# iiscleap/ICL-speech-text-LLM

Hardware: AMD Instinct MI355X
Metric: ICL utterances/sec (whole node), SALMONN+Llama2-7B 5-shot VOXCELEB (higher is better)
Workload: dtype bf16

## Files before the change

### icl-speech-text-llm_amd/csrc/gemm.hip

```cpp
#include "gemm_common.h"

using namespace iclg;

namespace {


#define TILE_STAGES_DEEP(BM_, BN_) (((BM_) + (BN_)) <= 128 ? 4 : 3)

template <int WAVES_M, int WAVES_N, int MI, int NI, int NST>
__global__ __launch_bounds__(256) void gemm_bf16_kernel(GemmParams p) {
  constexpr int BM = WAVES_M * MI * 16, BN = WAVES_N * NI * 16;
  constexpr int A_BYTES = BM * 128, W_BYTES = BN * 128, BUF = A_BYTES + W_BYTES;
  constexpr int A_INSTR = BM / 32, W_INSTR = BN / 32;
  constexpr int G_STAGE = A_INSTR + W_INSTR;
  static_assert(WAVES_M * WAVES_N == 4, "4 waves per block");
  extern __shared__ __attribute__((aligned(16))) char smem[];

  const int tid = threadIdx.x, lane = tid & 63;
  const int wave = __builtin_amdgcn_readfirstlane(tid >> 6);
  const int wm = wave / WAVES_N, wn = wave % WAVES_N;

  int tm, tn;
  block_to_tile(p, blockIdx.x, tm, tn);
  const int m0 = tm * BM, n0 = tn * BN;

  const int z = blockIdx.z;
  const __bf16* A = p.A;
  int kt0 = 0, kt1 = p.K >> 6;
  if (p.split_k > 1) {
    const int nk = p.K >> 6;
    kt0 = (int)(((int64_t)z * nk) / p.split_k);
    kt1 = (int)(((int64_t)(z + 1) * nk) / p.split_k);
  } else {
    A += (int64_t)z * p.sA;
  }

  const __bf16* ga[A_INSTR];
  const __bf16* gw[W_INSTR];
#pragma unroll
  for (int j = 0; j < A_INSTR; ++j) {
    const int row = (j * 4 + wave) * 8 + (lane >> 3);
    const int chunk = (lane & 7) ^ ((row >> 1) & 7);
    const int gm = min(m0 + row, p.M - 1);
    ga[j] = A + (int64_t)gm * p.lda + chunk * 8;
  }
#pragma unroll
  for (int j = 0; j < W_INSTR; ++j) {
    const int row = (j * 4 + wave) * 8 + (lane >> 3);
    const int chunk = (lane & 7) ^ ((row >> 1) & 7);
    const int gn = min(n0 + row, p.N - 1);
    gw[j] = p.W + (int64_t)gn * p.ldw + chunk * 8;
  }

  auto stage = [&](int buf_off, int kt) {
    char* base = smem + buf_off;
#pragma unroll
    for (int j = 0; j < A_INSTR; ++j)
      __builtin_amdgcn_global_load_lds((gptr_t)(ga[j] + (int64_t)kt * 64),
                                       (lptr_t)(base + (j * 4 + wave) * 1024), 16, 0, 0);
#pragma unroll
    for (int j = 0; j < W_INSTR; ++j)
      __builtin_amdgcn_global_load_lds((gptr_t)(gw[j] + (int64_t)kt * 64),
                                       (lptr_t)(base + A_BYTES + (j * 4 + wave) * 1024), 16, 0, 0);
  };

  const int fr = lane & 15, fq = lane >> 4;
  int a_off[2], w_off[2];
#pragma unroll
  for (int kk = 0; kk < 2; ++kk) {
    const int sw = ((kk * 4 + fq) ^ (fr >> 1)) * 16;
    a_off[kk] = (wm * MI * 16 + fr) * 128 + sw;
    w_off[kk] = (wn * NI * 16 + fr) * 128 + sw;
  }

  f32x4 acc[MI][NI];
#pragma unroll
  for (int i = 0; i < MI; ++i)
#pragma unroll
    for (int j = 0; j < NI; ++j) acc[i][j] = f32x4{0.f, 0.f, 0.f, 0.f};

  const bool vecp = p.split_k == 1 && vec_path_ok(p);
  const bool interior = vecp && (m0 + BM <= p.M) && (n0 + BN <= p.N);
  const bool fold_bias = vecp && (p.epi & ICL_EPI_BIAS);
// ... 41 lines not shown
          for (int j = 0; j < NI; ++j)
            acc[i][j] = __builtin_amdgcn_mfma_f32_16x16x32_bf16(wf[j], af[i], acc[i][j], 0, 0, 0);
      }
      fill = cur;
      cur = cur == (NST - 1) * BUF ? 0 : cur + BUF;
    }
    asm volatile("s_waitcnt vmcnt(0)" ::: "memory");
  }

  if (interior) {
    const int mb = m0 + wm * MI * 16 + fr, nb = n0 + wn * NI * 16 + fq * 4;
    if (p.epi & ICL_EPI_SWIGLU) {
      if constexpr (NI % 2 == 0) {
#pragma unroll
        for (int i = 0; i < MI; ++i)
#pragma unroll
          for (int j = 0; j < NI; j += 2) {
            f32x4 v;
#pragma unroll
            for (int r = 0; r < 4; ++r) v[r] = silu_f(acc[i][j][r]) * acc[i][j + 1][r];
            store_out4(p, (int64_t)z * p.sC + (int64_t)(mb + i * 16) * p.ldc + ((n0 + wn * NI * 16 + j * 16) >> 1) + fq * 4, v);
          }
      }
      return;
    }
    const bool late_res = p.epi & ICL_EPI_RESIDUAL;
    f32x4 rv[MI][NI];
    if (late_res) {
#pragma unroll
      for (int i = 0; i < MI; ++i)
#pragma unroll
        for (int j = 0; j < NI; ++j)
          rv[i][j] = load_res4(p, (int64_t)z * p.sR + (int64_t)(mb + i * 16) * p.ldr + nb + j * 16);
    }
#pragma unroll
    for (int i = 0; i < MI; ++i)
#pragma unroll
      for (int j = 0; j < NI; ++j) {
        f32x4 v = acc[i][j];
        if (p.epi & ICL_EPI_GELU) {
            v = gelu_erf4(v);
        }
        if (late_res) v = v + rv[i][j];
        store_out4(p, (int64_t)z * p.sC + (int64_t)(mb + i * 16) * p.ldc + nb + j * 16, v);
      }
    return;
  }
  GemmParams q = p;
  if (fold_bias) q.epi &= ~ICL_EPI_BIAS;
#pragma unroll
  for (int i = 0; i < MI; ++i) {
    const int m = m0 + wm * MI * 16 + i * 16 + fr;
#pragma unroll
    for (int j = 0; j < NI; ++j) {
      const int nt = n0 + wn * NI * 16 + j * 16;
      if (p.split_k > 1) {
        epi_store_partial(p, z, m, nt + fq * 4, acc[i][j]);
      } else if (p.epi & ICL_EPI_SWIGLU) {
        if constexpr (NI % 2 == 0) {
          if ((j & 1) == 0) epi_store_swiglu(q, z, m, nt, fq * 4, acc[i][j], acc[i][j + 1]);
        }
      } else {
        epi_store4(q, z, m, nt + fq * 4, acc[i][j]);
      }
    }
  }
}

__device__ __forceinline__ f32x4 sum_slabs4(const float* src, int64_t slab, int split) {
  f32x4 v = {0.f, 0.f, 0.f, 0.f};
  int s = 0;
  for (; s + 4 <= split; s += 4) {
    const f32x4 a = *(const f32x4*)(src + (s + 0) * slab), b = *(const f32x4*)(src + (s + 1) * slab);
    const f32x4 c = *(const f32x4*)(src + (s + 2) * slab), d = *(const f32x4*)(src + (s + 3) * slab);
    v = v + a;
    v = v + b;
    v = v + c;
    v = v + d;
  }
  for (; s < split; ++s) v = v + *(const f32x4*)(src + s * slab);
  return v;
}

__global__ __launch_bounds__(256) void gemm_splitk_reduce_kernel(GemmParams p) {
  const bool swiglu = p.epi & ICL_EPI_SWIGLU;
  const int Nout = swiglu ? p.N / 2 : p.N;
  const int64_t total = (int64_t)p.M * Nout;
  const int64_t slab = (int64_t)p.M * p.N;
  const bool vec = (p.N & 31) == 0 && (p.ldc & 3) == 0 && (!(p.epi & ICL_EPI_RESIDUAL) || ((p.ldr & 3) == 0 && p.res_dtype == ICL_F32)) &&
                   (((uintptr_t)p.ws | (uintptr_t)p.C) & 15) == 0 && (!(p.epi & ICL_EPI_BIAS) || ((uintptr_t)p.bias & 15) == 0) &&
                   (!(p.epi & ICL_EPI_RESIDUAL) || ((uintptr_t)p.R & 15) == 0);
  if (vec) {
    const int nq = Nout >> 2;
    const int64_t total4 = (int64_t)p.M * nq;
    for (int64_t idx = (int64_t)blockIdx.x * blockDim.x + threadIdx.x; idx < total4; idx += (int64_t)gridDim.x * blockDim.x) {
      const int m = (int)(idx / nq), c = (int)(idx % nq) * 4;
      f32x4 v;
      if (swiglu) {
        const int ng = (c >> 4) * 32 + (c & 15), nu = ng + 16;
        f32x4 g = sum_slabs4(p.ws + (int64_t)m * p.N + ng, slab, p.split_k);
        f32x4 u = sum_slabs4(p.ws + (int64_t)m * p.N + nu, slab, p.split_k);
        if (p.epi & ICL_EPI_BIAS) {
          g = g + *(const f32x4*)(p.bias + ng);
          u = u + *(const f32x4*)(p.bias + nu);
        }
#pragma unroll
        for (int r = 0; r < 4; ++r) v[r] = silu_f(g[r]) * u[r];
      } else {
        v = sum_slabs4(p.ws + (int64_t)m * p.N + c, slab, p.split_k);
        if (p.epi & ICL_EPI_BIAS) v = v + *(const f32x4*)(p.bias + c);
        if (p.epi & ICL_EPI_GELU) v = gelu_erf4(v);
        if (p.epi & ICL_EPI_RESIDUAL) v = v + *(const f32x4*)((const float*)p.R + (int64_t)m * p.ldr + c);
      }
      const int64_t coff = (int64_t)m * p.ldc + c;
      if (p.out_dtype == ICL_BF16) *(u32x2*)((unsigned short*)p.C + coff) = u32x2{pack_bf16x2(v[0], v[1]), pack_bf16x2(v[2], v[3])};
      else *(f32x4*)((float*)p.C + coff) = v;
    }
    return;
  }
  for (int64_t idx = (int64_t)blockIdx.x * blockDim.x + threadIdx.x; idx < total;
       idx += (int64_t)gridDim.x * blockDim.x) {
    const int m = (int)(idx / Nout), c = (int)(idx % Nout);
    float v;
    if (swiglu) {
      const int ng = (c >> 4) * 32 + (c & 15), nu = ng + 16;
      float g = 0.f, u = 0.f;
      for (int s = 0; s < p.split_k; ++s) {
        g += p.ws[s * slab + (int64_t)m * p.N + ng];
        u += p.ws[s * slab + (int64_t)m * p.N + nu];
      }
      if (p.epi & ICL_EPI_BIAS) {
        g += p.bias[ng];
        u += p.bias[nu];
      }
      v = silu_f(g) * u;
    } else {
      v = 0.f;
      for (int s = 0; s < p.split_k; ++s) v += p.ws[s * slab + (int64_t)m * p.N + c];
      if (p.epi & ICL_EPI_BIAS) v += p.bias[c];
      if (p.epi & ICL_EPI_GELU) v = gelu_erf(v);
      if (p.epi & ICL_EPI_RESIDUAL) {
        const int64_t roff = (int64_t)m * p.ldr + c;
        v += (p.res_dtype == ICL_F32) ? ((const float*)p.R)[roff]
                                      : bf16_bits_to_f32(((const unsigned short*)p.R)[roff]);
      }
    }
    const int64_t coff = (int64_t)m * p.ldc + c;
    if (p.out_dtype == ICL_BF16)
      ((unsigned short*)p.C)[coff] = f32_to_bf16_bits(v);
    else
      ((float*)p.C)[coff] = v;
  }
}



template <int VPT>
__global__ __launch_bounds__(256) void splitk_reduce_rmsnorm_kernel(GemmParams p, const float* gamma, float eps,
                                                                    unsigned short* xn, int64_t ldx) {
  __shared__ float wsum[4];
  const int m = blockIdx.x, tid = threadIdx.x, nvec = p.N >> 2;
  const int64_t slab = (int64_t)p.M * p.N;
  const bool store_c = p.split_k > 1 || p.ws != (const float*)p.C;
  f32x4 v[VPT];
#pragma unroll
  for (int i = 0; i < VPT; ++i) {
    const int c = tid + i * 256;
    v[i] = f32x4{0.f, 0.f, 0.f, 0.f};
    if (c < nvec) v[i] = sum_slabs4(p.ws + (int64_t)m * p.N + c * 4, slab, p.split_k);
  }
  float ss = 0.f;
#pragma unroll
  for (int i = 0; i < VPT; ++i) {
    const int c = tid + i * 256;
    if (c < nvec) {
      if (p.epi & ICL_EPI_RESIDUAL) v[i] = v[i] + *(const f32x4*)((const float*)p.R + (int64_t)m * p.ldr + c * 4);
      if (store_c) *(f32x4*)((float*)p.C + (int64_t)m * p.ldc + c * 4) = v[i];
      ss += v[i][0] * v[i][0] + v[i][1] * v[i][1] + v[i][2] * v[i][2] + v[i][3] * v[i][3];
    }
  }
  ss = wave_reduce_sum(ss);
  if ((tid & 63) == 0) wsum[tid >> 6] = ss;
  __syncthreads();
  const float rstd = rsqrtf((((wsum[0] + wsum[1]) + wsum[2]) + wsum[3]) / (float)p.N + eps);
#pragma unroll
  for (int i = 0; i < VPT; ++i) {
    const int c = tid + i * 256;
    if (c < nvec) {
      const f32x4 g = *(const f32x4*)(gamma + c * 4);
      const f32x4 o = v[i] * rstd * g;
      *(u32x2*)(xn + (int64_t)m * ldx + c * 4) = u32x2{pack_bf16x2(o[0], o[1]), pack_bf16x2(o[2], o[3])};
    }
  }
}


template <int WAVES_M, int WAVES_N, int MI, int NI, int NST>
int launch_tile_n(GemmParams& p, dim3 grid, hipStream_t stream) {
  constexpr int BM = WAVES_M * MI * 16, BN = WAVES_N * NI * 16;
  constexpr int SMEM = (BM + BN) * 128 * NST;
  if (const int rc = allow_dynamic_lds<gemm_bf16_kernel<WAVES_M, WAVES_N, MI, NI, NST>>(SMEM)) return rc;
  hipLaunchKernelGGL((gemm_bf16_kernel<WAVES_M, WAVES_N, MI, NI, NST>), grid, dim3(256), SMEM, stream, p);
  ICL_CHECK_LAUNCH("icl_gemm_bf16");
  return ICL_OK;
}

template <int WAVES_M, int WAVES_N, int MI, int NI>
int launch_tile(GemmParams& p, int batch, hipStream_t stream) {
  constexpr int BM = WAVES_M * MI * 16, BN = WAVES_N * NI * 16;
  constexpr int DEEP = TILE_STAGES_DEEP(BM, BN);
  p.tiles_m = (p.M + BM - 1) / BM;
  p.tiles_n = (p.N + BN - 1) / BN;
  dim3 grid(p.tiles_m * p.tiles_n, 1, p.split_k > 1 ? p.split_k : batch);
  static int n_cu = 0;
  if (n_cu <= 0) {
    n_cu = icl_device_cu_count();
    if (n_cu <= 0) n_cu = 256;
  }
  const int64_t blocks = (int64_t)grid.x * grid.z;
  const int per_cu = (160 * 1024) / ((BM + BN) * 128 * DEEP);
  if (blocks <= (int64_t)n_cu * per_cu) return launch_tile_n<WAVES_M, WAVES_N, MI, NI, DEEP>(p, grid, stream);
  return launch_tile_n<WAVES_M, WAVES_N, MI, NI, 2>(p, grid, stream);
}

struct NormFuse {
  const float* gamma;
  float eps;
  unsigned short* xn;
  int64_t ldx;
};

void launch_reduce_rmsnorm(const GemmParams& p, const NormFuse& nf, hipStream_t stream) {
  auto kern = p.N <= 4096 ? splitk_reduce_rmsnorm_kernel<4> : splitk_reduce_rmsnorm_kernel<8>;
  hipLaunchKernelGGL(kern, dim3(p.M), dim3(256), 0, stream, p, nf.gamma, nf.eps, nf.xn, nf.ldx);
}

}


extern "C" int icl_gemm_select_tile(int32_t M, int32_t N, int32_t K, int32_t batch, int32_t split_k) {
  const int64_t t128 = (int64_t)((M + 127) / 128) * ((N + 127) / 128) * batch;
  if (split_k > 1 || M <= 64 || t128 < 256) return 2;
  if (N <= 64) return 2;
  if (N <= 128) return 1;
  static int ncu = 0;
  if (ncu <= 0) {
    ncu = icl_device_cu_count();
    if (ncu <= 0) ncu = 256;
  }
  const int64_t t256 = (int64_t)((M + 255) / 256) * ((N + 255) / 256) * batch;
  const int64_t rounds = (t256 + ncu - 1) / ncu;
  const double eff = (double)t256 / (double)(rounds * ncu);
  if (K >= 768 && eff >= 0.6) return 3;
  return 1;
}

static int gemm_impl(const icl_gemm_args* a, void* stream_, const RopeFuse* rope, const NormFuse* norm = nullptr,
                     const float* wscale = nullptr) {
  hipStream_t stream = (hipStream_t)stream_;
  ICL_CHECK_ARG(a != nullptr, "icl_gemm_bf16: args is NULL");
  ICL_CHECK_ARG(a->A && a->W && a->C, "icl_gemm_bf16: A/W/C must be non-NULL");
  ICL_CHECK_ARG(a->M > 0 && a->N > 0 && a->K > 0, "icl_gemm_bf16: M,N,K must be > 0 (got %d,%d,%d)",
                a->M, a->N, a->K);
  ICL_CHECK_ARG(a->K % 64 == 0, "icl_gemm_bf16: K=%d must be a multiple of 64", a->K);
  ICL_CHECK_ARG(a->lda % 8 == 0 && a->ldw % 8 == 0,
                "icl_gemm_bf16: lda=%lld / ldw=%lld must be multiples of 8", (long long)a->lda,
                (long long)a->ldw);
  ICL_CHECK_ARG(((uintptr_t)a->A & 15) == 0 && ((uintptr_t)a->W & 15) == 0,
                "icl_gemm_bf16: A and W must be 16-byte aligned");
  ICL_CHECK_ARG(a->ldw >= a->K, "icl_gemm_bf16: ldw=%lld < K=%d", (long long)a->ldw, a->K);
  ICL_CHECK_ARG(a->batch >= 1 && a->batch <= 65535, "icl_gemm_bf16: batch=%d out of range", a->batch);
  ICL_CHECK_ARG(a->split_k >= 1 && a->split_k <= 64, "icl_gemm_bf16: split_k=%d out of range", a->split_k);
  ICL_CHECK_ARG(a->out_dtype == ICL_BF16 || a->out_dtype == ICL_F32, "icl_gemm_bf16: bad out_dtype %d",
                a->out_dtype);
  ICL_CHECK_ARG(a->res_dtype == ICL_BF16 || a->res_dtype == ICL_F32, "icl_gemm_bf16: bad res_dtype %d",
                a->res_dtype);
  ICL_CHECK_ARG((a->epilogue & ~15) == 0, "icl_gemm_bf16: unknown epilogue bits 0x%x", a->epilogue);
  const bool swiglu = a->epilogue & ICL_EPI_SWIGLU;
  if (swiglu) {
    ICL_CHECK_ARG(a->N % 32 == 0, "icl_gemm_bf16: SWIGLU needs N %% 32 == 0 (N=%d)", a->N);
    ICL_CHECK_ARG((a->epilogue & (ICL_EPI_GELU | ICL_EPI_RESIDUAL)) == 0,
                  "icl_gemm_bf16: SWIGLU cannot be combined with GELU/RESIDUAL");
    ICL_CHECK_ARG(a->ldc % 4 == 0, "icl_gemm_bf16: SWIGLU needs ldc %% 4 == 0");
  }
  if (a->epilogue & ICL_EPI_BIAS) ICL_CHECK_ARG(a->bias, "icl_gemm_bf16: EPI_BIAS without bias");
  if (a->epilogue & ICL_EPI_RESIDUAL) ICL_CHECK_ARG(a->R, "icl_gemm_bf16: EPI_RESIDUAL without R");
  const int nout = swiglu ? a->N / 2 : a->N;
  ICL_CHECK_ARG(a->ldc >= nout, "icl_gemm_bf16: ldc=%lld < %d output columns", (long long)a->ldc, nout);
  if (a->split_k > 1) {
    ICL_CHECK_ARG(a->batch == 1, "icl_gemm_bf16: split_k > 1 requires batch == 1");
    ICL_CHECK_ARG(a->workspace, "icl_gemm_bf16: split_k > 1 requires a workspace");
    ICL_CHECK_ARG(a->split_k <= a->K / 64, "icl_gemm_bf16: split_k=%d > K/64=%d", a->split_k, a->K / 64);
  }
  const int cal = a->out_dtype == ICL_BF16 ? 8 : 16;
  ICL_CHECK_ARG(((uintptr_t)a->C % cal) == 0, "icl_gemm_bf16: C must be %d-byte aligned", cal);
  if (a->R) {
    const int ral = a->res_dtype == ICL_BF16 ? 8 : 16;
    ICL_CHECK_ARG(((uintptr_t)a->R % ral) == 0, "icl_gemm_bf16: R must be %d-byte aligned", ral);
  }

  GemmParams p;
  p.A = (const __bf16*)a->A;
  p.W = (const __bf16*)a->W;
  p.C = a->C;
  p.bias = a->bias;
  p.R = a->R;
  p.ws = a->workspace;
  p.lda = a->lda; p.ldw = a->ldw; p.ldc = a->ldc; p.ldr = a->ldr;
  p.sA = a->strideA; p.sC = a->strideC; p.sR = a->strideR;
  p.M = a->M; p.N = a->N; p.K = a->K;
  p.epi = a->epilogue; p.out_dtype = a->out_dtype; p.res_dtype = a->res_dtype;
  p.split_k = a->split_k;
  p.tiles_m = p.tiles_n = 0;
  p.group_m = p.xcd_sync = 0;

  if (!rope && (wscale || a->tile == 4 || a->tile == 6)) {
    if (!(a->M <= 64 && a->batch == 1)) {
      if (wscale) icl_set_error("icl_gemm_fp8w: needs M <= 64 and batch == 1 (M=%d batch=%d)", a->M, a->batch);
      else icl_set_error("icl_gemm_bf16: the skinny kernel needs M <= 64 and batch == 1");
      return ICL_EINVAL;
    }
    p.split_k = 1;
    return launch_skinny(p, wscale ? SKINNY_W_FP8 : a->tile == 6 ? SKINNY_W_PACKED : SKINNY_W_ROW, wscale, stream);
  }
  int tile = a->tile;
  if (tile == 0) tile = icl_gemm_select_tile(a->M, a->N, a->K, a->batch, a->split_k);
  if (tile == 3 && a->K < 128) tile = 1;
  if (rope) {
    ICL_CHECK_ARG(tile == 3, "icl_gemm_rope_kv_bf16: only the 256x256 tile fuses RoPE (this problem resolves to tile %d; "
                             "use icl_gemm_bf16 + icl_rope_kv_bf16)", tile);
    ICL_CHECK_ARG(a->split_k == 1, "icl_gemm_rope_kv_bf16: split_k must be 1");
    return launch_tile256(p, 1, stream, rope);
  }
  int rc;
  if (tile == 1)
    rc = launch_tile<2, 2, 4, 4>(p, a->batch, stream);
  else if (tile == 2)
    rc = launch_tile<2, 2, 2, 2>(p, a->batch, stream);
  else if (tile == 3) {
    ICL_CHECK_ARG(a->split_k == 1 || (a->split_k <= a->K / 128 && a->N % 4 == 0),
                  "icl_gemm_bf16: split_k=%d on the 256x256 tile needs K / split_k >= 128 and N %% 4 == 0 (K=%d N=%d)", a->split_k, a->K, a->N);
    rc = launch_tile256(p, a->batch, stream);
  } else if (tile == 5) {
    ICL_CHECK_ARG(a->M <= 256 && a->batch == 1, "icl_gemm_bf16: the decode tile needs M <= 256 and batch == 1");
    rc = launch_decode_tile(p, stream);
  } else {
    icl_set_error("icl_gemm_bf16: unsupported tile id %d", tile);
    return ICL_EINVAL;
  }
  if (rc != ICL_OK) return rc;
  if (a->split_k > 1 && norm) {
    launch_reduce_rmsnorm(p, *norm, stream);
    ICL_CHECK_LAUNCH("icl_gemm_rmsnorm_bf16(split-K reduce + RMSNorm)");
  } else if (a->split_k > 1) {
    const int64_t total = (int64_t)a->M * nout;
    int blocks = (int)((total + 255) / 256);
    if (blocks > 2048) blocks = 2048;
    hipLaunchKernelGGL(gemm_splitk_reduce_kernel, dim3(blocks), dim3(256), 0, stream, p);
    ICL_CHECK_LAUNCH("icl_gemm_bf16(split-K reduce)");
  }
  return ICL_OK;
}

extern "C" int icl_rmsnorm(const void* x, int64_t ldx, const float* gamma, void* y, int64_t ldy, int32_t M, int32_t N, float eps,
                           int32_t in_dtype, int32_t out_dtype, void* stream);

static int gemm_rmsnorm_impl(const icl_gemm_args* a, const float* wscale, const float* gamma, float eps, void* xn, int64_t ld_xn,
                             void* stream) {
  ICL_CHECK_ARG(a != nullptr && gamma && xn, "icl_gemm_rmsnorm_bf16: NULL pointer");
  ICL_CHECK_ARG(a->batch == 1 && a->out_dtype == ICL_F32 && (a->epilogue & ~ICL_EPI_RESIDUAL) == 0 &&
                    (!(a->epilogue & ICL_EPI_RESIDUAL) || a->res_dtype == ICL_F32),
                "icl_gemm_rmsnorm_bf16: batch 1, f32 output, residual-only epilogue with an f32 residual");
  ICL_CHECK_ARG(a->N % 4 == 0 && a->N <= 8192 && a->ldc % 4 == 0 && a->ldr % 4 == 0 && ld_xn % 4 == 0 && ld_xn >= a->N,
                "icl_gemm_rmsnorm_bf16: N=%d must be a multiple of 4 and <= 8192, leading dimensions multiples of 4", a->N);
  ICL_CHECK_ARG(((uintptr_t)gamma & 15) == 0 && ((uintptr_t)xn & 7) == 0 && ((uintptr_t)a->C & 15) == 0 &&
                    (!a->R || ((uintptr_t)a->R & 15) == 0), "icl_gemm_rmsnorm_bf16: misaligned pointer");
  if (a->split_k > 1 && a->tile != 4 && a->tile != 6 && !wscale) {
    const NormFuse nf{gamma, eps, (unsigned short*)xn, ld_xn};
    return gemm_impl(a, stream, nullptr, &nf);
  }
  const int rc = gemm_impl(a, stream, nullptr, nullptr, wscale);
  if (rc != ICL_OK) return rc;
#ifndef ICL_SMALL_M_BLOCKNORM
#define ICL_SMALL_M_BLOCKNORM 1
#endif
  if (ICL_SMALL_M_BLOCKNORM && a->M <= 64 && a->ldc == a->N) {
    GemmParams q{};
    q.ws = (float*)a->C; q.C = a->C; q.R = nullptr; q.ldc = a->ldc; q.ldr = 0; q.M = a->M; q.N = a->N; q.split_k = 1; q.epi = 0;
    launch_reduce_rmsnorm(q, NormFuse{gamma, eps, (unsigned short*)xn, ld_xn}, (hipStream_t)stream);
    ICL_CHECK_LAUNCH("icl_gemm_rmsnorm_bf16(row-per-block RMSNorm)");
    return ICL_OK;
  }
  return icl_rmsnorm(a->C, a->ldc, gamma, xn, ld_xn, a->M, a->N, eps, ICL_F32, ICL_BF16, stream);
}

extern "C" int icl_gemm_rmsnorm_bf16(const icl_gemm_args* a, const float* gamma, float eps, void* xn, int64_t ld_xn, void* stream) {
  return gemm_rmsnorm_impl(a, nullptr, gamma, eps, xn, ld_xn, stream);
}

extern "C" int icl_gemm_bf16(const icl_gemm_args* a, void* stream) { return gemm_impl(a, stream, nullptr); }

extern "C" int icl_gemm_fp8w(const icl_gemm_args* a, const float* w_scale, void* stream) {
  ICL_CHECK_ARG(w_scale, "icl_gemm_fp8w: w_scale is NULL");
  return gemm_impl(a, stream, nullptr, nullptr, w_scale);
}

extern "C" int icl_gemm_rmsnorm_fp8w(const icl_gemm_args* a, const float* w_scale, const float* gamma, float eps, void* xn,
                                     int64_t ld_xn, void* stream) {
  ICL_CHECK_ARG(w_scale, "icl_gemm_rmsnorm_fp8w: w_scale is NULL");
  return gemm_rmsnorm_impl(a, w_scale, gamma, eps, xn, ld_xn, stream);
}

extern "C" int icl_gemm_rope_kv_bf16(const icl_gemm_args* a, int64_t k_off, int64_t v_off, const float* cosT,
                                     const float* sinT, const int32_t* pos, const int32_t* seq_ids, void* kcache,
                                     void* vcache, int32_t n_heads, int32_t head_dim, int32_t max_len, int32_t kv_rows_to_c,
                                     void* stream) {
  ICL_CHECK_ARG(a != nullptr && cosT && sinT && pos, "icl_gemm_rope_kv_bf16: NULL pointer");
  ICL_CHECK_ARG(head_dim == 128, "icl_gemm_rope_kv_bf16: head_dim=%d (the fused epilogue is built for 128)", head_dim);
  const int64_t hd = (int64_t)n_heads * 128;
  ICL_CHECK_ARG(n_heads > 0 && hd % 256 == 0 && (k_off == 0 || k_off == hd) && (v_off == k_off || v_off == k_off + hd) &&
                    (a->N == v_off || a->N == v_off + hd) && a->N > 0,
                "icl_gemm_rope_kv_bf16: need q|k|v blocks of n_heads*128 columns each (or empty), a multiple of 256 (N=%d k_off=%lld v_off=%lld)",
                a->N, (long long)k_off, (long long)v_off);
  ICL_CHECK_ARG(a->batch == 1 && a->out_dtype == ICL_BF16 && (a->epilogue & ~ICL_EPI_BIAS) == 0,
                "icl_gemm_rope_kv_bf16: batch 1, bf16 output, bias-only epilogue");
  ICL_CHECK_ARG(a->C && ((uintptr_t)a->C & 15) == 0 && a->ldc % 8 == 0, "icl_gemm_rope_kv_bf16: C must be 16-byte aligned, ldc %% 8 == 0");
  ICL_CHECK_ARG(!a->bias || ((uintptr_t)a->bias & 15) == 0, "icl_gemm_rope_kv_bf16: bias must be 16-byte aligned");
  ICL_CHECK_ARG(((uintptr_t)cosT & 15) == 0 && ((uintptr_t)sinT & 15) == 0, "icl_gemm_rope_kv_bf16: cos/sin misaligned");
  ICL_CHECK_ARG((kcache == nullptr) == (vcache == nullptr), "icl_gemm_rope_kv_bf16: kcache and vcache must both be set or both NULL");
  if (kcache) {
    ICL_CHECK_ARG(seq_ids && max_len > 0, "icl_gemm_rope_kv_bf16: cache append needs seq_ids and max_len");
    ICL_CHECK_ARG(((uintptr_t)kcache & 15) == 0 && ((uintptr_t)vcache & 15) == 0, "icl_gemm_rope_kv_bf16: cache misaligned");
  }
  ICL_CHECK_ARG(kv_rows_to_c || kcache, "icl_gemm_rope_kv_bf16: kv_rows_to_c = 0 needs a cache to hold k / v");
  RopeFuse rf;
  rf.kv_rows_to_c = kv_rows_to_c;
  rf.cosT = cosT; rf.sinT = sinT; rf.pos = pos; rf.seq_ids = seq_ids;
  rf.kc = (unsigned short*)kcache; rf.vc = (unsigned short*)vcache;
  rf.k_off = (int)k_off; rf.v_off = (int)v_off; rf.H = n_heads; rf.max_len = max_len;
  return gemm_impl(a, stream, &rf);
}
// ... 1 lines not shown
```

### icl-speech-text-llm_amd/csrc/gemm256.hip

```cpp
#include "gemm_common.h"
#include <cstdlib>

using namespace iclg;

#ifndef ICL_EPI_NT
#define ICL_EPI_NT 3
#endif

namespace {

constexpr int T256_REGION = 128 * 128;
constexpr int T256_BUF = 4 * T256_REGION;
constexpr int T256_SMEM = 256 * (256 * 2 + 16);

__device__ __forceinline__ void st16(unsigned short* dst, u32x4 v) {
  if (ICL_EPI_NT & 4) __builtin_nontemporal_store(v, (u32x4*)dst);
  else *(u32x4*)dst = v;
}

__device__ __forceinline__ void rope_rows(const GemmParams& p, const RopeFuse& rf, const char* smem, int pitch, int m0,
                                          int n0, int tid) {
  const int sect = n0 >= rf.v_off ? 2 : (n0 >= rf.k_off ? 1 : 0);
  const int head0 = (n0 - (sect == 2 ? rf.v_off : sect == 1 ? rf.k_off : 0)) >> 7;
  unsigned short* C = (unsigned short*)p.C;
  constexpr int U = 4;
  if (sect == 2) {
    for (int base = tid; base < 256 * 32; base += U * 512) {
      int64_t crow[U];
      if (rf.vc) {
#pragma unroll
        for (int u = 0; u < U; ++u) {
          const int m = min(m0 + ((base + u * 512) >> 5), p.M - 1);
          crow[u] = (int64_t)rf.seq_ids[m] * rf.H * rf.max_len + rf.pos[m];
        }
      }
#pragma unroll
      for (int u = 0; u < U; ++u) {
        const int c = base + u * 512, row = c >> 5, cc = c & 31, m = m0 + row;
        if (m >= p.M) continue;
        const u32x4 v = *(const u32x4*)(smem + row * pitch + cc * 16);
        if (rf.kv_rows_to_c) st16(C + (int64_t)m * p.ldc + n0 + cc * 8, v);
        if (rf.vc) st16(rf.vc + (crow[u] + (int64_t)(head0 + (cc >> 4)) * rf.max_len) * 128 + (cc & 15) * 8, v);
      }
    }
    return;
  }
  const bool to_cache = sect == 1 && rf.kc;
  for (int base = tid; base < 256 * 16; base += U * 512) {
    int ps[U], sq[U];
    u32x4 lo[U], hi[U];
    f32x4 c0[U], c1[U], s0[U], s1[U];
#pragma unroll
    for (int u = 0; u < U; ++u) {
      const int m = min(m0 + ((base + u * 512) >> 4), p.M - 1);
      ps[u] = rf.pos[m];
      sq[u] = to_cache ? rf.seq_ids[m] : 0;
    }
#pragma unroll
    for (int u = 0; u < U; ++u) {
      const int it = base + u * 512, row = it >> 4, hh = (it >> 3) & 1, j = it & 7;
      const char* src = smem + row * pitch + hh * 256 + j * 16;
      lo[u] = *(const u32x4*)src;
      hi[u] = *(const u32x4*)(src + 128);
      const float* cp = rf.cosT + (int64_t)ps[u] * 64 + j * 8;
      const float* sp = rf.sinT + (int64_t)ps[u] * 64 + j * 8;
      c0[u] = *(const f32x4*)cp;
      c1[u] = *(const f32x4*)(cp + 4);
      s0[u] = *(const f32x4*)sp;
      s1[u] = *(const f32x4*)(sp + 4);
    }
#pragma unroll
    for (int u = 0; u < U; ++u) {
      const int it = base + u * 512, row = it >> 4, hh = (it >> 3) & 1, j = it & 7, m = m0 + row;
      if (m >= p.M) continue;
      u32x4 olo, ohi;
      rope_rot8(lo[u], hi[u], c0[u], c1[u], s0[u], s1[u], olo, ohi);
      if (sect == 0 || rf.kv_rows_to_c) {
        unsigned short* dst = C + (int64_t)m * p.ldc + n0 + hh * 128 + j * 8;
        st16(dst, olo);
        st16(dst + 64, ohi);
      }
      if (to_cache) {
        unsigned short* cd = rf.kc + (((int64_t)sq[u] * rf.H + head0 + hh) * rf.max_len + ps[u]) * 128 + j * 8;
        st16(cd, olo);
        st16(cd + 64, ohi);
      }
    }
  }
}

constexpr int T256_OUT_F32 = 16;
template <bool ROPE, int EPI>
__global__ __launch_bounds__(512, 2) void gemm256_bf16_kernel(GemmParams p_in, RopeFuse rf) {
  GemmParams p = p_in;
  p.epi = (p_in.epi & ICL_EPI_BIAS) | (EPI & (ICL_EPI_GELU | ICL_EPI_RESIDUAL | ICL_EPI_SWIGLU));
  p.out_dtype = (EPI & T256_OUT_F32) ? ICL_F32 : ICL_BF16;
  extern __shared__ __attribute__((aligned(16))) char smem[];
  const int tid = threadIdx.x, lane = tid & 63;
  const int wave = __builtin_amdgcn_readfirstlane(tid >> 6);
  const int wr = wave >> 2, wc = wave & 3;
  int tm, tn;
  block_to_tile(p, blockIdx.x, tm, tn);
  const int m0 = tm * 256, n0 = tn * 256;
  int z = blockIdx.z;
  int nk = p.K >> 6, kt0 = 0;
  const bool slab_out = p.split_k > 1;
  if (p.split_k > 1) {
    kt0 = (int)(((int64_t)z * nk) / p.split_k);
    nk = (int)(((int64_t)(z + 1) * nk) / p.split_k) - kt0;
    p.C = p.ws + (int64_t)z * p.M * p.N;
    p.ldc = p.N;
    p.sC = 0;
    p.epi = 0;
    z = 0;
  }
  const __bf16* A = p.A + (int64_t)z * p.sA + (int64_t)kt0 * 64;
  const __bf16* Wk = p.W + (int64_t)kt0 * 64;

  const __bf16* gsrc[2][2][2];
#pragma unroll
  for (int h = 0; h < 2; ++h)
#pragma unroll
    for (int r = 0; r < 2; ++r) {
      const int row = (r * 8 + wave) * 8 + (lane >> 3);
      const int chunk = (lane & 7) ^ ((row >> 1) & 7);
      gsrc[0][h][r] = A + (int64_t)min(m0 + h * 128 + row, p.M - 1) * p.lda + chunk * 8;
      gsrc[1][h][r] = Wk + (int64_t)min(n0 + h * 128 + row, p.N - 1) * p.ldw + chunk * 8;
    }
  auto stage = [&](int bo, int which, int h, int kt) {
    const int64_t koff = (int64_t)min(kt, nk - 1) * 64;
    char* base = smem + bo + (which * 2 + h) * T256_REGION + wave * 1024;
    __builtin_amdgcn_global_load_lds((gptr_t)(gsrc[which][h][0] + koff), (lptr_t)(base), 16, 0, 0);
    __builtin_amdgcn_global_load_lds((gptr_t)(gsrc[which][h][1] + koff), (lptr_t)(base + 8 * 1024), 16, 0, 0);
  };

  const int fr = lane & 15, fq = lane >> 4;
  const int a_base = (wr * 64 + fr) * 128, b_base = (wc * 32 + fr) * 128;
  const int sw0 = ((0 + fq) ^ (fr >> 1)) * 16, sw1 = ((4 + fq) ^ (fr >> 1)) * 16;

  f32x4 acc[2][2][4][2];
#pragma unroll
  for (int a = 0; a < 2; ++a)
#pragma unroll
    for (int b = 0; b < 2; ++b)
#pragma unroll
      for (int i = 0; i < 4; ++i)
#pragma unroll
        for (int j = 0; j < 2; ++j) acc[a][b][i][j] = f32x4{0.f, 0.f, 0.f, 0.f};
  bf16x8 af[4][2], b0f[2][2], b1f[2][2];
  const bool vecp = vec_path_ok(p);
  const bool interior = vecp && (m0 + 256 <= p.M) && (n0 + 256 <= p.N);
  const bool fold_bias = vecp && (p.epi & ICL_EPI_BIAS);
  constexpr bool fold_res = false;

  auto read_a = [&](int bo, int h) {
    const char* r = smem + bo + h * T256_REGION + a_base;
#pragma unroll
    for (int i = 0; i < 4; ++i) {
      af[i][0] = *(const bf16x8*)(r + i * 2048 + sw0);
      af[i][1] = *(const bf16x8*)(r + i * 2048 + sw1);
    }
  };
  auto read_b = [&](int bo, int h, bf16x8 (&bf)[2][2]) {
    const char* r = smem + bo + (2 + h) * T256_REGION + b_base;
#pragma unroll
    for (int j = 0; j < 2; ++j) {
      bf[j][0] = *(const bf16x8*)(r + j * 2048 + sw0);
      bf[j][1] = *(const bf16x8*)(r + j * 2048 + sw1);
    }
  };
  auto mma = [&](f32x4 (&c)[4][2], bf16x8 (&bf)[2][2]) {
    __builtin_amdgcn_s_setprio(1);
#pragma unroll
    for (int kk = 0; kk < 2; ++kk)
// ... 21 lines not shown
  auto tile = [&](int bo, int t, auto mode) {
    constexpr int MODE = decltype(mode)::value;
    const int bx = bo ^ T256_BUF;
    read_a(bo, 0);
    read_b(bo, 0, b0f);
    if constexpr (MODE != 2) stage(bx, 1, 1, t + 1);
    phase_sync(std::integral_constant<int, MODE == 2 ? 2 : 8>{});
    mma(acc[0][0], b0f);
    read_b(bo, 1, b1f);
    if constexpr (MODE != 2) stage(bx, 0, 1, t + 1);
    phase_sync(std::integral_constant<int, MODE == 2 ? 0 : 8>{});
    mma(acc[0][1], b1f);
    read_a(bo, 1);
    if constexpr (MODE == 0) stage(bo, 0, 0, t + 2);
    phase_sync(std::integral_constant<int, MODE == 0 ? 8 : (MODE == 1 ? 6 : 0)>{});
    mma(acc[1][1], b1f);
    if constexpr (MODE == 0) stage(bo, 1, 0, t + 2);
    phase_sync(std::integral_constant<int, MODE == 0 ? 8 : (MODE == 1 ? 4 : 0)>{});
    mma(acc[1][0], b0f);
  };
  using M0_ = std::integral_constant<int, 0>;
  using M1_ = std::integral_constant<int, 1>;
  using M2_ = std::integral_constant<int, 2>;

  f32x4 bias_f[2][2];
  if (fold_res) {
#pragma unroll
    for (int qa = 0; qa < 2; ++qa)
#pragma unroll
      for (int qb = 0; qb < 2; ++qb)
#pragma unroll
        for (int i = 0; i < 4; ++i)
#pragma unroll
          for (int j = 0; j < 2; ++j) {
            const int m = m0 + qa * 128 + wr * 64 + i * 16 + fr, n = n0 + qb * 128 + wc * 32 + j * 16 + fq * 4;
            if (interior || (m < p.M && n < p.N))
              acc[qa][qb][i][j] = *(const f32x4*)((const float*)p.R + (int64_t)z * p.sR + (int64_t)m * p.ldr + n);
          }
  }
  if (fold_bias) {
#pragma unroll
    for (int qb = 0; qb < 2; ++qb)
#pragma unroll
      for (int j = 0; j < 2; ++j) {
        const int n = n0 + qb * 128 + wc * 32 + j * 16 + fq * 4;
        bias_f[qb][j] = (interior || n < p.N) ? *(const f32x4*)(p.bias + n) : f32x4{0.f, 0.f, 0.f, 0.f};
      }
  }
  __builtin_amdgcn_sched_barrier(0);
  stage(0, 0, 0, 0);
  stage(0, 1, 0, 0);
  stage(0, 1, 1, 0);
  stage(0, 0, 1, 0);
  stage(T256_BUF, 0, 0, 1);
  stage(T256_BUF, 1, 0, 1);
  __builtin_amdgcn_sched_barrier(0);
  if (fold_bias) {
#pragma unroll
    for (int qa = 0; qa < 2; ++qa)
#pragma unroll
      for (int qb = 0; qb < 2; ++qb)
#pragma unroll
        for (int i = 0; i < 4; ++i)
#pragma unroll
          for (int j = 0; j < 2; ++j) acc[qa][qb][i][j] = acc[qa][qb][i][j] + bias_f[qb][j];
  }
  phase_sync(std::integral_constant<int, 8>{});
  if (wr == 1) __builtin_amdgcn_s_barrier();
  const int n_steady = nk - 2;
  int t = 0;
  for (; t + 1 < n_steady; t += 2) {
    tile(0, t, M0_{});
    tile(T256_BUF, t + 1, M0_{});
  }
  if (t < n_steady) {
    tile(0, t, M0_{});
    ++t;
  }
  const int bo = (t & 1) ? T256_BUF : 0;
  tile(bo, t, M1_{});
  tile(bo ^ T256_BUF, t + 1, M2_{});
  if (wr == 0) __builtin_amdgcn_s_barrier();

  const int es_out = p.out_dtype == ICL_BF16 ? 2 : 4;
  const bool rows16 = (((uintptr_t)p.C | (uintptr_t)(p.ldc * es_out) | (uintptr_t)(p.sC * es_out)) & 15) == 0;
  const bool has_res = p.epi & ICL_EPI_RESIDUAL;
  const bool res_rows = has_res && p.res_dtype == ICL_F32 && p.out_dtype == ICL_F32 && !(p.epi & ICL_EPI_SWIGLU) &&
                        (((uintptr_t)p.R | (uintptr_t)(p.ldr * 4) | (uintptr_t)(p.sR * 4)) & 15) == 0;
  if (ROPE || (interior && rows16 && (!has_res || res_rows))) {
    const bool swiglu = p.epi & ICL_EPI_SWIGLU;
    const bool obf = p.out_dtype == ICL_BF16;
    const int out_cols = swiglu ? 128 : 256;
    const int es = obf ? 2 : 4;
    const int pitch = out_cols * es + 16;
    const int chunks_per_row = out_cols * es / 16;
    const int64_t c_col0 = swiglu ? (n0 >> 1) : n0;
    const bool one_round = ROPE || obf;
    f32x4 rrA[16], rrB[16];
    auto load_res_rows = [&](int qa_, f32x4 (&rr)[16]) {
      const char* rbase = (const char*)p.R + ((int64_t)z * p.sR + (int64_t)(m0 + qa_ * 128) * p.ldr + n0) * 4;
#pragma unroll
      for (int it = 0; it < 16; ++it) {
        const int c = tid + it * 512, row = c >> 6, cc = c & 63;
        rr[it] = ICL_EPI_NT & 1 ? __builtin_nontemporal_load((const f32x4*)(rbase + (int64_t)row * p.ldr * 4 + cc * 16))
                                : *(const f32x4*)(rbase + (int64_t)row * p.ldr * 4 + cc * 16);
      }
    };
    if (has_res) load_res_rows(0, rrA);
#pragma unroll
    for (int qa = 0; qa < 2; ++qa) {
      if (qa == 0 || !one_round) __syncthreads();
      const int row_off = one_round ? qa * 128 : 0;
#pragma unroll
      for (int qb = 0; qb < 2; ++qb)
#pragma unroll
        for (int i = 0; i < 4; ++i) {
          const int row = row_off + wr * 64 + i * 16 + fr;
          if (swiglu) {
            f32x4 v;
#pragma unroll
            for (int r = 0; r < 4; ++r) v[r] = silu_f(acc[qa][qb][i][0][r]) * acc[qa][qb][i][1][r];
            const int col = qb * 64 + wc * 16 + fq * 4;
            char* dst = smem + row * pitch + col * es;
            if (obf) *(u32x2*)dst = u32x2{pack_bf16x2(v[0], v[1]), pack_bf16x2(v[2], v[3])};
            else *(f32x4*)dst = v;
          } else {
#pragma unroll
            for (int j = 0; j < 2; ++j) {
              f32x4 v = acc[qa][qb][i][j];
              if (p.epi & ICL_EPI_GELU) {
            v = gelu_erf4(v);
              }
              const int col = qb * 128 + wc * 32 + j * 16 + fq * 4;
              char* dst = smem + row * pitch + col * es;
              if (obf) *(u32x2*)dst = u32x2{pack_bf16x2(v[0], v[1]), pack_bf16x2(v[2], v[3])};
              else *(f32x4*)dst = v;
            }
          }
        }
      if (one_round && qa == 0) continue;
      __syncthreads();
      if constexpr (ROPE) {
        rope_rows(p, rf, smem, pitch, m0, n0, tid);
        continue;
      }
      char* cbase = (char*)p.C + ((int64_t)z * p.sC + (int64_t)(m0 + (one_round ? 0 : qa * 128)) * p.ldc + c_col0) * es;
      const int n_chunks = (one_round ? 256 : 128) * chunks_per_row;
      if (has_res) {
        if (qa == 0) load_res_rows(1, rrB);
        f32x4 (&rr)[16] = qa == 0 ? rrA : rrB;
#pragma unroll
        for (int it = 0; it < 16; ++it) {
          const int c = tid + it * 512, row = c >> 6, cc = c & 63;
          const f32x4 v = *(const f32x4*)(smem + row * pitch + cc * 16) + rr[it];
          if (ICL_EPI_NT & 1) __builtin_nontemporal_store(v, (f32x4*)(cbase + (int64_t)row * p.ldc * 4 + cc * 16));
          else *(f32x4*)(cbase + (int64_t)row * p.ldc * 4 + cc * 16) = v;
        }
      } else {
        const int n_iter = n_chunks >> 9;
        u32x4 v[16];
#pragma unroll
        for (int it = 0; it < 16; ++it)
          if (it < n_iter) {
            const int c = tid + it * 512, row = c / chunks_per_row, cc = c - row * chunks_per_row;
            v[it] = *(const u32x4*)(smem + row * pitch + cc * 16);
          }
// ... 17 lines not shown
        for (int i = 0; i < 4; ++i)
#pragma unroll
          for (int qb = 0; qb < 2; ++qb) {
            f32x4 v;
#pragma unroll
            for (int r = 0; r < 4; ++r) v[r] = silu_f(acc[qa][qb][i][0][r]) * acc[qa][qb][i][1][r];
            store_out4(p, (int64_t)z * p.sC + (int64_t)(mb + i * 16) * p.ldc + ((n0 + qb * 128 + wc * 32) >> 1) + fq * 4, v);
          }
        continue;
      }
      f32x4 rv[2][4][2];
      if (late_res) {
#pragma unroll
        for (int qb = 0; qb < 2; ++qb)
#pragma unroll
          for (int i = 0; i < 4; ++i)
#pragma unroll
            for (int j = 0; j < 2; ++j)
              rv[qb][i][j] = load_res4(p, (int64_t)z * p.sR + (int64_t)(mb + i * 16) * p.ldr + n0 + qb * 128 + wc * 32 + j * 16 + fq * 4);
      }
#pragma unroll
      for (int qb = 0; qb < 2; ++qb)
#pragma unroll
        for (int i = 0; i < 4; ++i)
#pragma unroll
          for (int j = 0; j < 2; ++j) {
            f32x4 v = acc[qa][qb][i][j];
            if (p.epi & ICL_EPI_GELU) {
            v = gelu_erf4(v);
            }
            if (late_res) v = v + rv[qb][i][j];
            store_out4(p, (int64_t)z * p.sC + (int64_t)(mb + i * 16) * p.ldc + n0 + qb * 128 + wc * 32 + j * 16 + fq * 4, v);
          }
    }
    return;
  }

  GemmParams q = p;
  if (fold_bias) q.epi &= ~ICL_EPI_BIAS;
  if (fold_res) q.epi &= ~ICL_EPI_RESIDUAL;
#pragma unroll
  for (int qa = 0; qa < 2; ++qa)
#pragma unroll
    for (int i = 0; i < 4; ++i) {
      const int m = m0 + qa * 128 + wr * 64 + i * 16 + fr;
#pragma unroll
      for (int qb = 0; qb < 2; ++qb) {
        const int nt = n0 + qb * 128 + wc * 32;
        if (p.epi & ICL_EPI_SWIGLU) {
          epi_store_swiglu(q, z, m, nt, fq * 4, acc[qa][qb][i][0], acc[qa][qb][i][1]);
        } else {
          epi_store4(q, z, m, nt + fq * 4, acc[qa][qb][i][0]);
          epi_store4(q, z, m, nt + 16 + fq * 4, acc[qa][qb][i][1]);
        }
      }
    }
}

template <bool ROPE, int EPI>
int launch256(const GemmParams& p, const dim3& grid, hipStream_t stream, const RopeFuse& rf) {
  auto kern = gemm256_bf16_kernel<ROPE, EPI>;
  if (const int rc = allow_dynamic_lds<gemm256_bf16_kernel<ROPE, EPI>>(T256_SMEM)) return rc;
  hipLaunchKernelGGL(kern, grid, dim3(512), T256_SMEM, stream, p, rf);
  ICL_CHECK_LAUNCH("icl_gemm_bf16(256)");
  return ICL_OK;
}

}

int iclg::launch_tile256(GemmParams& p, int batch, hipStream_t stream, const RopeFuse* rope) {
  p.tiles_m = (p.M + 255) / 256;
  p.tiles_n = (p.N + 255) / 256;
  {
    static const int env_gm = [] { const char* e = getenv("ICL_GEMM_GROUP_M"); return e ? atoi(e) : 0; }();
    static const int env_xs = [] { const char* e = getenv("ICL_GEMM_XCD_SYNC"); return e ? atoi(e) : 1; }();
    const int64_t panel = (int64_t)256 * p.K * 2;
    p.group_m = env_gm > 0 ? env_gm : (int)std::min<int64_t>(6, std::max<int64_t>(1, 8400000 / panel));
    p.xcd_sync = env_xs;
  }
  const dim3 grid(p.tiles_m * p.tiles_n, 1, p.split_k > 1 ? p.split_k : batch);
  if (rope) return launch256<true, 0>(p, grid, stream, *rope);
  const RopeFuse none{};
  constexpr int G = ICL_EPI_GELU, R = ICL_EPI_RESIDUAL, S = ICL_EPI_SWIGLU, F = T256_OUT_F32;
  if (p.split_k > 1) return launch256<false, F>(p, grid, stream, none);
  switch ((p.epi & (G | R | S)) | (p.out_dtype == ICL_F32 ? F : 0)) {
    case 0:         return launch256<false, 0>(p, grid, stream, none);
    case G:         return launch256<false, G>(p, grid, stream, none);
    case R:         return launch256<false, R>(p, grid, stream, none);
    case G | R:     return launch256<false, G | R>(p, grid, stream, none);
    case S:         return launch256<false, S>(p, grid, stream, none);
    case F:         return launch256<false, F>(p, grid, stream, none);
    case F | G:     return launch256<false, F | G>(p, grid, stream, none);
    case F | R:     return launch256<false, F | R>(p, grid, stream, none);
    case F | G | R: return launch256<false, F | G | R>(p, grid, stream, none);
    case F | S:     return launch256<false, F | S>(p, grid, stream, none);
  }
  icl_set_error("icl_gemm_bf16(256): unsupported epilogue combination 0x%x", p.epi);
  return ICL_EINVAL;
}
```

### icl-speech-text-llm_amd/csrc/gemm_common.h

```cpp
#pragma once
#include "common.h"
#include <algorithm>
#include <type_traits>

namespace iclg {


struct GemmParams {
  const __bf16* A;
  const __bf16* W;
  void* C;
  const float* bias;
  const void* R;
  float* ws;
  int64_t lda, ldw, ldc, ldr, sA, sC, sR;
  int M, N, K, epi, out_dtype, res_dtype, split_k, tiles_m, tiles_n;
  int group_m;
  int xcd_sync;
};

constexpr int GROUP_M = 8;

typedef const __attribute__((address_space(1))) void* gptr_t;
typedef __attribute__((address_space(3))) void* lptr_t;


__device__ __forceinline__ void epi_store4(const GemmParams& p, int z, int m, int n, f32x4 acc) {
  if (m >= p.M || n >= p.N) return;
  const bool has_bias = p.epi & ICL_EPI_BIAS, has_gelu = p.epi & ICL_EPI_GELU, has_res = p.epi & ICL_EPI_RESIDUAL;
  char* Cb = (char*)p.C;
  const int64_t cz = (int64_t)z * p.sC, rz = (int64_t)z * p.sR;
  const bool vec_ok = ((p.ldc & 3) == 0) && (!has_res || (p.ldr & 3) == 0);
  float v[4] = {acc[0], acc[1], acc[2], acc[3]};
  const bool full = (n + 3 < p.N);
  if (has_bias) {
#pragma unroll
    for (int r = 0; r < 4; ++r)
      if (full || n + r < p.N) v[r] += p.bias[n + r];
  }
  if (has_gelu) {
    const f32x4 g = gelu_erf4(f32x4{v[0], v[1], v[2], v[3]});
#pragma unroll
    for (int r = 0; r < 4; ++r) v[r] = g[r];
  }
  const int64_t coff = cz + (int64_t)m * p.ldc + n;
  if (full && vec_ok) {
    if (has_res) {
      const int64_t roff = rz + (int64_t)m * p.ldr + n;
      if (p.res_dtype == ICL_F32) {
        f32x4 rv = *(const f32x4*)((const char*)p.R + roff * 4);
#pragma unroll
        for (int r = 0; r < 4; ++r) v[r] += rv[r];
      } else {
        const unsigned short* rp = (const unsigned short*)p.R + roff;
#pragma unroll
        for (int r = 0; r < 4; ++r) v[r] += bf16_bits_to_f32(rp[r]);
      }
    }
    if (p.out_dtype == ICL_BF16) {
      u32x2 pk = {pack_bf16x2(v[0], v[1]), pack_bf16x2(v[2], v[3])};
      *(u32x2*)(Cb + coff * 2) = pk;
    } else {
      *(f32x4*)(Cb + coff * 4) = f32x4{v[0], v[1], v[2], v[3]};
    }
  } else {
#pragma unroll
    for (int r = 0; r < 4; ++r) {
      if (n + r >= p.N) continue;
      float x = v[r];
      if (has_res) {
        const int64_t roff = rz + (int64_t)m * p.ldr + n + r;
        x += (p.res_dtype == ICL_F32) ? ((const float*)p.R)[roff]
                                      : bf16_bits_to_f32(((const unsigned short*)p.R)[roff]);
      }
      if (p.out_dtype == ICL_BF16)
        ((unsigned short*)Cb)[coff + r] = f32_to_bf16_bits(x);
      else
        ((float*)Cb)[coff + r] = x;
    }
  }
}
__device__ __forceinline__ void epi_store_swiglu(const GemmParams& p, int z, int m, int nt, int fq4, f32x4 g4, f32x4 u4) {
  if (m >= p.M || nt >= p.N) return;
  float v[4];
#pragma unroll
  for (int r = 0; r < 4; ++r) {
    float g = g4[r], u = u4[r];
    if (p.epi & ICL_EPI_BIAS) {
      g += p.bias[nt + fq4 + r];
      u += p.bias[nt + 16 + fq4 + r];
    }
    v[r] = silu_f(g) * u;
  }
  const int64_t off = (int64_t)z * p.sC + (int64_t)m * p.ldc + (nt >> 1) + fq4;
  if (p.out_dtype == ICL_BF16) {
    u32x2 pk = {pack_bf16x2(v[0], v[1]), pack_bf16x2(v[2], v[3])};
    *(u32x2*)((char*)p.C + off * 2) = pk;
  } else {
    *(f32x4*)((char*)p.C + off * 4) = f32x4{v[0], v[1], v[2], v[3]};
  }
}
__device__ __forceinline__ void epi_store_partial(const GemmParams& p, int z, int m, int n, f32x4 acc) {
  if (m >= p.M || n >= p.N) return;
  float* dst = p.ws + (int64_t)z * p.M * p.N + (int64_t)m * p.N + n;
// ... 90 lines not shown
```

Baseline: 144.6.

## Store split-K partials in column-blocked slab layout and batch RMSNorm rows per block

The 256x256 split-K GEMM now writes its fp32 partial tiles into a column-blocked (16-column panel) workspace layout through a dedicated epilogue, instead of row-major through the generic F32 epilogue. The split-K reduce and reduce+RMSNorm kernels read that layout, and the reduce kernel walks indices in 4-row by 16-quad blocks. The RMSNorm reduce handles two rows per block. The goal is contiguous, coalesced 64-byte segments on both the partial store and the reduce read. It is on by default, with an environment variable to turn it off, and adds more kernel template instances and indexing arithmetic.

```diff
diff --git a/icl-speech-text-llm_amd/csrc/gemm.hip b/icl-speech-text-llm_amd/csrc/gemm.hip
--- a/icl-speech-text-llm_amd/csrc/gemm.hip
+++ b/icl-speech-text-llm_amd/csrc/gemm.hip
@@ -1,4 +1,5 @@
 #include "gemm_common.h"
+#include <cstdlib>
 
 using namespace iclg;
 
@@ -206,6 +207,7 @@
   return v;
 }
 
+template <bool TILED>
 __global__ __launch_bounds__(256) void gemm_splitk_reduce_kernel(GemmParams p) {
   const bool swiglu = p.epi & ICL_EPI_SWIGLU;
   const int Nout = swiglu ? p.N / 2 : p.N;
@@ -216,14 +218,24 @@
                    (!(p.epi & ICL_EPI_RESIDUAL) || ((uintptr_t)p.R & 15) == 0);
   if (vec) {
     const int nq = Nout >> 2;
-    const int64_t total4 = (int64_t)p.M * nq;
+    const int nqb = (nq + 15) >> 4, nrb = (p.M + 3) >> 2;
+    const int64_t total4 = TILED ? (int64_t)nrb * nqb * 64 : (int64_t)p.M * nq;
     for (int64_t idx = (int64_t)blockIdx.x * blockDim.x + threadIdx.x; idx < total4; idx += (int64_t)gridDim.x * blockDim.x) {
-      const int m = (int)(idx / nq), c = (int)(idx % nq) * 4;
+      int m, c;
+      if constexpr (TILED) {
+        const int blk = (int)(idx >> 6), in = (int)idx & 63;
+        m = (blk % nrb) * 4 + (in >> 4);
+        c = ((blk / nrb) * 16 + (in & 15)) * 4;
+        if (m >= p.M || c >= Nout) continue;
+      } else {
+        m = (int)(idx / nq);
+        c = (int)(idx % nq) * 4;
+      }
       f32x4 v;
       if (swiglu) {
         const int ng = (c >> 4) * 32 + (c & 15), nu = ng + 16;
-        f32x4 g = sum_slabs4(p.ws + (int64_t)m * p.N + ng, slab, p.split_k);
-        f32x4 u = sum_slabs4(p.ws + (int64_t)m * p.N + nu, slab, p.split_k);
+        f32x4 g = sum_slabs4(p.ws + slab_index<TILED>(m, ng, p.M, p.N), slab, p.split_k);
+        f32x4 u = sum_slabs4(p.ws + slab_index<TILED>(m, nu, p.M, p.N), slab, p.split_k);
         if (p.epi & ICL_EPI_BIAS) {
           g = g + *(const f32x4*)(p.bias + ng);
           u = u + *(const f32x4*)(p.bias + nu);
@@ -231,7 +243,7 @@
 #pragma unroll
         for (int r = 0; r < 4; ++r) v[r] = silu_f(g[r]) * u[r];
       } else {
-        v = sum_slabs4(p.ws + (int64_t)m * p.N + c, slab, p.split_k);
+        v = sum_slabs4(p.ws + slab_index<TILED>(m, c, p.M, p.N), slab, p.split_k);
         if (p.epi & ICL_EPI_BIAS) v = v + *(const f32x4*)(p.bias + c);
         if (p.epi & ICL_EPI_GELU) v = gelu_erf4(v);
         if (p.epi & ICL_EPI_RESIDUAL) v = v + *(const f32x4*)((const float*)p.R + (int64_t)m * p.ldr + c);
@@ -250,8 +262,8 @@
       const int ng = (c >> 4) * 32 + (c & 15), nu = ng + 16;
       float g = 0.f, u = 0.f;
       for (int s = 0; s < p.split_k; ++s) {
-        g += p.ws[s * slab + (int64_t)m * p.N + ng];
-        u += p.ws[s * slab + (int64_t)m * p.N + nu];
+        g += p.ws[s * slab + slab_index<TILED>(m, ng, p.M, p.N)];
+        u += p.ws[s * slab + slab_index<TILED>(m, nu, p.M, p.N)];
       }
       if (p.epi & ICL_EPI_BIAS) {
         g += p.bias[ng];
@@ -260,7 +272,7 @@
       v = silu_f(g) * u;
     } else {
       v = 0.f;
-      for (int s = 0; s < p.split_k; ++s) v += p.ws[s * slab + (int64_t)m * p.N + c];
+      for (int s = 0; s < p.split_k; ++s) v += p.ws[s * slab + slab_index<TILED>(m, c, p.M, p.N)];
       if (p.epi & ICL_EPI_BIAS) v += p.bias[c];
       if (p.epi & ICL_EPI_GELU) v = gelu_erf(v);
       if (p.epi & ICL_EPI_RESIDUAL) {
@@ -279,11 +291,15 @@
 
 
 
-template <int VPT>
-__global__ __launch_bounds__(256) void splitk_reduce_rmsnorm_kernel(GemmParams p, const float* gamma, float eps,
-                                                                    unsigned short* xn, int64_t ldx) {
-  __shared__ float wsum[4];
-  const int m = blockIdx.x, tid = threadIdx.x, nvec = p.N >> 2;
+#ifndef ICL_RMS_TILED_ROWS
+#define ICL_RMS_TILED_ROWS 2
+#endif
+template <int VPT, bool TILED, int ROWS>
+__global__ __launch_bounds__(256 * ROWS) void splitk_reduce_rmsnorm_kernel(GemmParams p, const float* gamma, float eps,
+                                                                           unsigned short* xn, int64_t ldx) {
+  __shared__ float wsum[ROWS][4];
+  const int row = threadIdx.x >> 8, tid = threadIdx.x & 255, m = blockIdx.x * ROWS + row;
+  const int nvec = m < p.M ? p.N >> 2 : 0;
   const int64_t slab = (int64_t)p.M * p.N;
   const bool store_c = p.split_k > 1 || p.ws != (const float*)p.C;
   f32x4 v[VPT];
@@ -291,7 +307,7 @@
   for (int i = 0; i < VPT; ++i) {
     const int c = tid + i * 256;
     v[i] = f32x4{0.f, 0.f, 0.f, 0.f};
-    if (c < nvec) v[i] = sum_slabs4(p.ws + (int64_t)m * p.N + c * 4, slab, p.split_k);
+    if (c < nvec) v[i] = sum_slabs4(p.ws + slab_index<TILED>(m, c * 4, p.M, p.N), slab, p.split_k);
   }
   float ss = 0.f;
 #pragma unroll
@@ -304,9 +320,9 @@
     }
   }
   ss = wave_reduce_sum(ss);
-  if ((tid & 63) == 0) wsum[tid >> 6] = ss;
+  if ((tid & 63) == 0) wsum[row][tid >> 6] = ss;
   __syncthreads();
-  const float rstd = rsqrtf((((wsum[0] + wsum[1]) + wsum[2]) + wsum[3]) / (float)p.N + eps);
+  const float rstd = rsqrtf((((wsum[row][0] + wsum[row][1]) + wsum[row][2]) + wsum[row][3]) / (float)p.N + eps);
 #pragma unroll
   for (int i = 0; i < VPT; ++i) {
     const int c = tid + i * 256;
@@ -355,7 +371,13 @@
 };
 
 void launch_reduce_rmsnorm(const GemmParams& p, const NormFuse& nf, hipStream_t stream) {
-  auto kern = p.N <= 4096 ? splitk_reduce_rmsnorm_kernel<4> : splitk_reduce_rmsnorm_kernel<8>;
+  constexpr int TR = ICL_RMS_TILED_ROWS;
+  if (p.slab_tiled) {
+    auto kern = p.N <= 4096 ? splitk_reduce_rmsnorm_kernel<4, true, TR> : splitk_reduce_rmsnorm_kernel<8, true, TR>;
+    hipLaunchKernelGGL(kern, dim3((p.M + TR - 1) / TR), dim3(256 * TR), 0, stream, p, nf.gamma, nf.eps, nf.xn, nf.ldx);
+    return;
+  }
+  auto kern = p.N <= 4096 ? splitk_reduce_rmsnorm_kernel<4, false, 1> : splitk_reduce_rmsnorm_kernel<8, false, 1>;
   hipLaunchKernelGGL(kern, dim3(p.M), dim3(256), 0, stream, p, nf.gamma, nf.eps, nf.xn, nf.ldx);
 }
 
@@ -437,6 +459,7 @@
   p.split_k = a->split_k;
   p.tiles_m = p.tiles_n = 0;
   p.group_m = p.xcd_sync = 0;
+  p.slab_tiled = 0;
 
   if (!rope && (wscale || a->tile == 4 || a->tile == 6)) {
     if (!(a->M <= 64 && a->batch == 1)) {
@@ -464,6 +487,10 @@
   else if (tile == 3) {
     ICL_CHECK_ARG(a->split_k == 1 || (a->split_k <= a->K / 128 && a->N % 4 == 0),
                   "icl_gemm_bf16: split_k=%d on the 256x256 tile needs K / split_k >= 128 and N %% 4 == 0 (K=%d N=%d)", a->split_k, a->K, a->N);
+    if (a->split_k > 1 && a->N % 16 == 0 && a->N % SLAB_COLS == 0 && ((uintptr_t)a->workspace & 15) == 0 && !(norm && a->split_k > 8)) {
+      const char* e = getenv("ICL_GEMM_SLAB_ROWS");
+      p.slab_tiled = !(e && atoi(e) != 0);
+    }
     rc = launch_tile256(p, a->batch, stream);
   } else if (tile == 5) {
     ICL_CHECK_ARG(a->M <= 256 && a->batch == 1, "icl_gemm_bf16: the decode tile needs M <= 256 and batch == 1");
@@ -480,7 +507,8 @@
     const int64_t total = (int64_t)a->M * nout;
     int blocks = (int)((total + 255) / 256);
     if (blocks > 2048) blocks = 2048;
-    hipLaunchKernelGGL(gemm_splitk_reduce_kernel, dim3(blocks), dim3(256), 0, stream, p);
+    if (p.slab_tiled) hipLaunchKernelGGL(gemm_splitk_reduce_kernel<true>, dim3(blocks), dim3(256), 0, stream, p);
+    else hipLaunchKernelGGL(gemm_splitk_reduce_kernel<false>, dim3(blocks), dim3(256), 0, stream, p);
     ICL_CHECK_LAUNCH("icl_gemm_bf16(split-K reduce)");
   }
   return ICL_OK;
diff --git a/icl-speech-text-llm_amd/csrc/gemm256.hip b/icl-speech-text-llm_amd/csrc/gemm256.hip
--- a/icl-speech-text-llm_amd/csrc/gemm256.hip
+++ b/icl-speech-text-llm_amd/csrc/gemm256.hip
@@ -90,6 +90,7 @@
 }
 
 constexpr int T256_OUT_F32 = 16;
+constexpr int T256_SLAB_TILED = 32;
 template <bool ROPE, int EPI>
 __global__ __launch_bounds__(512, 2) void gemm256_bf16_kernel(GemmParams p_in, RopeFuse rf) {
   GemmParams p = p_in;
@@ -277,6 +278,24 @@
   tile(bo ^ T256_BUF, t + 1, M2_{});
   if (wr == 0) __builtin_amdgcn_s_barrier();
 
+  if constexpr ((EPI & T256_SLAB_TILED) != 0) {
+    float* slab = (float*)p.C;
+#pragma unroll
+    for (int qb = 0; qb < 2; ++qb)
+#pragma unroll
+      for (int j = 0; j < 2; ++j) {
+        const int n = n0 + qb * 128 + wc * 32 + j * 16 + fq * 4;
+#pragma unroll
+        for (int qa = 0; qa < 2; ++qa)
+#pragma unroll
+          for (int i = 0; i < 4; ++i) {
+            const int m = m0 + qa * 128 + wr * 64 + i * 16 + fr;
+            if (m < p.M && n < p.N) *(f32x4*)(slab + slab_index<true>(m, n, p.M, p.N)) = acc[qa][qb][i][j];
+          }
+      }
+    return;
+  }
+
   const int es_out = p.out_dtype == ICL_BF16 ? 2 : 4;
   const bool rows16 = (((uintptr_t)p.C | (uintptr_t)(p.ldc * es_out) | (uintptr_t)(p.sC * es_out)) & 15) == 0;
   const bool has_res = p.epi & ICL_EPI_RESIDUAL;
@@ -460,8 +479,8 @@
   if (rope) return launch256<true, 0>(p, grid, stream, *rope);
   const RopeFuse none{};
   constexpr int G = ICL_EPI_GELU, R = ICL_EPI_RESIDUAL, S = ICL_EPI_SWIGLU, F = T256_OUT_F32;
-  if (p.split_k > 1) return launch256<false, F>(p, grid, stream, none);
-  switch ((p.epi & (G | R | S)) | (p.out_dtype == ICL_F32 ? F : 0)) {
+  if (p.split_k > 1 && !p.slab_tiled) return launch256<false, F>(p, grid, stream, none);
+  if (p.split_k == 1) switch ((p.epi & (G | R | S)) | (p.out_dtype == ICL_F32 ? F : 0)) {
     case 0:         return launch256<false, 0>(p, grid, stream, none);
     case G:         return launch256<false, G>(p, grid, stream, none);
     case R:         return launch256<false, R>(p, grid, stream, none);
@@ -473,6 +492,7 @@
     case F | G | R: return launch256<false, F | G | R>(p, grid, stream, none);
     case F | S:     return launch256<false, F | S>(p, grid, stream, none);
   }
+  if (p.split_k > 1) return launch256<false, F | T256_SLAB_TILED>(p, grid, stream, none);
   icl_set_error("icl_gemm_bf16(256): unsupported epilogue combination 0x%x", p.epi);
   return ICL_EINVAL;
 }
diff --git a/icl-speech-text-llm_amd/csrc/gemm_common.h b/icl-speech-text-llm_amd/csrc/gemm_common.h
--- a/icl-speech-text-llm_amd/csrc/gemm_common.h
+++ b/icl-speech-text-llm_amd/csrc/gemm_common.h
@@ -17,9 +17,20 @@
   int M, N, K, epi, out_dtype, res_dtype, split_k, tiles_m, tiles_n;
   int group_m;
   int xcd_sync;
+  int slab_tiled;
 };
 
 constexpr int GROUP_M = 8;
+
+#ifndef ICL_SLAB_COLS
+#define ICL_SLAB_COLS 16
+#endif
+constexpr int SLAB_COLS = ICL_SLAB_COLS;
+template <bool TILED>
+__host__ __device__ __forceinline__ int64_t slab_index(int m, int n, int M, int N) {
+  if constexpr (TILED) return ((int64_t)(n / SLAB_COLS) * M + m) * SLAB_COLS + n % SLAB_COLS;
+  else return (int64_t)m * N + n;
+}
 
 typedef const __attribute__((address_space(1))) void* gptr_t;
 typedef __attribute__((address_space(3))) void* lptr_t;
```

Result: no change. 144.7, median of 4 (+0.1%).
